# quarterwave0/LithographySimulator

Hardware: AMD Instinct MI355X
Metric: Abbe source-points x image-pixels per second (higher is better)
Workload: dtype f32

## Files before the change

### lithographysimulator_amd/csrc/engine_kernels.hpp

```cpp
#pragma once
#include <hip/hip_runtime.h>

#include "engine_common.hpp"
#include "abbe_plan.hpp"
#include "fft_core.hpp"
#include "wave_fft.hpp"

namespace litho {

template <int LOG2N>
struct Launch {
    using F = LineFFT<LOG2N, +1>;
    static constexpr int L = (F::T >= 64) ? 1 : 64 / F::T;
    static constexpr int THREADS = F::T * L;
#ifndef LITHO_NBUF
#define LITHO_NBUF 1
#endif
    static constexpr int NBUF = (LOG2N <= 12) ? LITHO_NBUF : 1;
    static constexpr size_t LDS_EXCH = (size_t)L * NBUF * F::LDS_LINE;
    static constexpr size_t LDS_BYTES = sizeof(float2) * (LDS_EXCH + F::LDS_TW);
#ifndef LITHO_WG_PER_CU
#define LITHO_WG_PER_CU 3
#endif
    static constexpr int WG_PER_CU = LOG2N <= 12 ? LITHO_WG_PER_CU : (LOG2N == 13 ? 2 : 1);
    static constexpr int WAVES = (THREADS / 256 > 0 ? THREADS / 256 : 1) * WG_PER_CU;
};


typedef unsigned int u32x2 __attribute__((ext_vector_type(2)));
static constexpr unsigned BUF_OOB = 0xFFFF0000u;

__device__ __forceinline__ __amdgpu_buffer_rsrc_t make_rsrc(const void* base, size_t bytes) {
    return __builtin_amdgcn_make_buffer_rsrc(const_cast<void*>(base), 0, (int)(unsigned)bytes, 0x00020000);
}
__device__ __forceinline__ float2 buf_load_c64(__amdgpu_buffer_rsrc_t r, unsigned off) {
    const u32x2 v = __builtin_amdgcn_raw_buffer_load_b64(r, off, 0, 0);
    return make_float2(__uint_as_float(v.x), __uint_as_float(v.y));
}
#ifndef LITHO_XSTORE_AUX
#define LITHO_XSTORE_AUX 16
#endif
template <int LOG2N> inline constexpr int t_store_aux = LOG2N >= 11 ? LITHO_XSTORE_AUX : 0;
typedef unsigned int u32x4 __attribute__((ext_vector_type(4)));
template <int AUX = 0>
__device__ __forceinline__ void buf_store_c64x2(__amdgpu_buffer_rsrc_t r, unsigned off, float2 a, float2 b) {
    u32x4 w;
    w.x = __float_as_uint(a.x); w.y = __float_as_uint(a.y);
    w.z = __float_as_uint(b.x); w.w = __float_as_uint(b.y);
    __builtin_amdgcn_raw_buffer_store_b128(w, r, off, 0, AUX);
}
template <int AUX = 0>
__device__ __forceinline__ void buf_store_c64(__amdgpu_buffer_rsrc_t r, unsigned off, float2 v) {
    u32x2 w;
    w.x = __float_as_uint(v.x);
    w.y = __float_as_uint(v.y);
    __builtin_amdgcn_raw_buffer_store_b64(w, r, off, 0, AUX);
}

__device__ __forceinline__ unsigned t_offset(const PassGeom& g, unsigned a, unsigned q) {
    return ((((q >> g.tcl) * g.rows + a) << g.tcl) + (q & ((1u << g.tcl) - 1u)));
}

typedef unsigned int uint2v __attribute__((ext_vector_type(2)));

__device__ __forceinline__ void touch_vgpr(float2& v) { asm volatile("" : "+v"(v.x), "+v"(v.y)); }
__device__ __forceinline__ void diag_keep(float2 v, unsigned o) { asm volatile("" ::"v"(v.x), "v"(v.y), "v"(o)); }

__device__ __forceinline__ const float* pack_weights() { return nullptr; }
__device__ __forceinline__ const float* pack_weights(const float* w) { return w; }

template <int LOG2N, int RL, bool PRUNED, int NP, int RP = 1, typename... Wt>
__global__ __launch_bounds__(Launch<LOG2N>::THREADS, (RP == 2 ? Launch<LOG2N>::WAVES / Launch<LOG2N>::WG_PER_CU * 2 : Launch<LOG2N>::WAVES)) void k_xpass_abbe(
    const float2* __restrict__ P, const float2* __restrict__ M, const int* __restrict__ shifts,
    float2* __restrict__ Tbuf, const float2* __restrict__ twtab, PassGeom g, int nb, int chunk, Wt... wts)
{
    constexpr bool WT = sizeof...(Wt) != 0;
    static_assert(sizeof...(Wt) <= 1 && !(WT && RP == 2), "weighted x-pass: one weight list, one row per workgroup (a weighted call ignores the row-pair knob)");
    [[maybe_unused]] const float* weights = pack_weights(wts...);
    using F = LineFFT<LOG2N, +1>;
    using LC = Launch<LOG2N>;
    constexpr unsigned IN = PRUNED ? natural_in_mask(RL) : 0xFFFFu;
    constexpr unsigned OUT = out_mask(RL);
    extern __shared__ __attribute__((aligned(16))) unsigned char smem_raw[];
    float2* smem = reinterpret_cast<float2*>(smem_raw);
    const int lt = threadIdx.x % F::T, lg = threadIdx.x / F::T;
    float2* lds = smem + (size_t)lg * LC::NBUF * F::LDS_LINE;

    typename F::Twiddles tw;
    F::load_twiddles(tw, twtab, lt, smem + LC::LDS_EXCH, threadIdx.x, LC::THREADS);

    static_assert(RP == 1 || (RP == 2 && NP == 1 && LC::L == 1), "row pairs: one plane, one line per workgroup");
    int a;
    if constexpr (LC::L == 1) {
        const int b = blockIdx.x, xcd = b & 7, i = b >> 3;
        a = ((i >> 2) * 32 + xcd * 4 + (i & 3)) * RP;
    } else {
        a = blockIdx.x * LC::L + lg;
    }
    const bool active = a < g.rows;
    const bool active1 = a + 1 < g.rows;
    const int r = g.ky0 + g.c + a;
    const size_t plane_bytes = (size_t)g.pn * g.pn * sizeof(float2);
    const __amdgpu_buffer_rsrc_t rM = make_rsrc(M, plane_bytes);

    unsigned koff[16];
    float2 pv[NP * RP][16];
    static_for<0, 16>([&](auto e_) {
        constexpr int e = decltype(e_)::value;
        if constexpr ((IN >> e) & 1u) {
            int k;
            const bool ok = centred_index(lt + F::T * e, F::N, g.kx0, g.kx1, k) && active;
            koff[e] = ok ? (unsigned)(g.c + k) : BUF_OOB;
        }
    });
    static_for<0, NP * RP>([&](auto p_) {
        constexpr int p = decltype(p_)::value;
        const __amdgpu_buffer_rsrc_t rP = make_rsrc(P + (size_t)(RP == 1 ? p : 0) * g.pn * g.pn, plane_bytes);
        static_for<0, 16>([&](auto e_) {
            constexpr int e = decltype(e_)::value;
            if constexpr ((IN >> e) & 1u)
                pv[p][e] = buf_load_c64(rP, koff[e] != BUF_OOB ? ((unsigned)(r + (RP == 1 ? 0 : p)) * g.pn + koff[e]) * 8u : BUF_OOB);
        });
    });
    unsigned toff[16];
    static_for<0, 16>([&](auto m_) {
        constexpr int m = decltype(m_)::value;
        if constexpr ((OUT >> m) & 1u) {
            int u;
            const bool ok = centred_index(lt + F::T * m, F::N, -g.c, g.pn - g.c, u) && active;
            const unsigned q = (unsigned)(u + g.c);
            toff[m] = ok ? t_offset(g, a, q) * 8u : BUF_OOB;
        }
    });

    const int s_begin = blockIdx.y * chunk;
    const int s_end = min(nb, s_begin + chunk);
    auto load_window = [&](int s, int rr, float2 (&mv)[16]) {
        const int dy = shifts[2 * s], dx = shifts[2 * s + 1];
        const unsigned mrow = (unsigned)(r + rr + dy) * g.pn + dx;
        static_for<0, 16>([&](auto e_) {
            constexpr int e = decltype(e_)::value;
            if constexpr ((IN >> e) & 1u)
#ifdef LITHO_DIAG_XNOLOAD
                mv[e] = make_float2((float)((mrow + koff[e]) & 1023u), 1.0f);
#else
                mv[e] = buf_load_c64(rM, koff[e] != BUF_OOB ? (mrow + koff[e]) * 8u : BUF_OOB);
#endif
        });
    };

    int flip = 0;
    float2 mnext[16];
    [[maybe_unused]] float wnext = 1.f;
    if (s_begin < s_end) load_window(s_begin, 0, mnext);
    if constexpr (WT) { if (s_begin < s_end) wnext = weights[s_begin]; }
    static_for<0, 16>([&](auto e_) {
        constexpr int e = decltype(e_)::value;
        if constexpr ((IN >> e) & 1u) touch_vgpr(mnext[e]);
    });
    const unsigned row1 = active1 ? (8u << g.tcl) : 0x80000000u;
    float2 held[RP == 2 ? 16 : 1];
    const bool hi8 = (threadIdx.x & 8) != 0;
    unsigned offc = 0, offd = 0;
    if constexpr (RP == 2) {
        const unsigned tileb = (unsigned)g.rows * (8u << g.tcl);
        offc = hi8 ? row1 - tileb : 0u;
        offd = hi8 ? 0u : row1 + tileb;
    }
    for (int s = s_begin; s < s_end; ++s) {
        static_for<0, RP>([&](auto rr_) {
            constexpr int rr = decltype(rr_)::value;
            float2 mv[16];
            static_for<0, 16>([&](auto e_) {
                constexpr int e = decltype(e_)::value;
                if constexpr ((IN >> e) & 1u) mv[e] = mnext[e];
            });
            [[maybe_unused]] float amp = 1.f;
            if constexpr (WT) amp = sqrtf(wnext);
#ifndef LITHO_XPASS_NO_PREFETCH
            if constexpr (rr + 1 < RP) load_window(s, rr + 1, mnext);
            else load_window(s + 1 < s_end ? s + 1 : s, 0, mnext);
#else
            if constexpr (rr + 1 < RP) load_window(s, rr + 1, mnext);
            else if (s + 1 < s_end) load_window(s + 1, 0, mnext);
#endif
            if constexpr (WT) {
                wnext = weights[s + 1 < s_end ? s + 1 : s];
                static_for<0, 16>([&](auto e_) {
                    constexpr int e = decltype(e_)::value;
                    if constexpr ((IN >> e) & 1u) mv[e] = make_float2(amp * mv[e].x, amp * mv[e].y);
                });
            }
            static_for<0, NP>([&](auto p_) {
                constexpr int p = decltype(p_)::value;
                float2 x[16];
                static_for<0, 16>([&](auto e_) {
                    constexpr int e = decltype(e_)::value;
                    if constexpr ((IN >> e) & 1u) x[e] = cmul(pv[RP == 1 ? p : rr][e], mv[e]);
                    else x[e] = make_float2(0.f, 0.f);
                });
                F::template run<LC::NBUF>(x, tw, lds, lt, flip);
                const __amdgpu_buffer_rsrc_t rT =
                    make_rsrc(Tbuf + ((size_t)p * nb + s) * g.t_point, (size_t)g.t_point * sizeof(float2));
                if constexpr (RP == 2 && rr == 0) {
                    static_for<0, 16>([&](auto m_) { held[decltype(m_)::value] = x[decltype(m_)::value]; });
                } else {
                    static_for<0, 16>([&](auto m_) {
                        constexpr int m = decltype(m_)::value;
#ifdef LITHO_DIAG_XNOSTORE
                        if constexpr ((OUT >> m) & 1u) diag_keep(x[m], toff[m]);
#elif defined(LITHO_DIAG_XSTORE_L2)
                        if constexpr ((OUT >> m) & 1u) buf_store_c64(rT, toff[m] == BUF_OOB ? BUF_OOB : (toff[m] & 0xFFFFFu), x[m]);
#else
                        if constexpr ((OUT >> m) & 1u) {
                            if constexpr (RP == 2) {
                                if (active) {
                                    const float bx = __uint_as_float(__builtin_amdgcn_update_dpp(0u, __float_as_uint(x[m].x), 0x128, 0xF, 0xF, false));
                                    const float by = __uint_as_float(__builtin_amdgcn_update_dpp(0u, __float_as_uint(x[m].y), 0x128, 0xF, 0xF, false));
                                    buf_store_c64<t_store_aux<LOG2N>>(rT, toff[m] + offc, hi8 ? make_float2(bx, by) : held[m]);
                                    buf_store_c64<t_store_aux<LOG2N>>(rT, toff[m] + offd, hi8 ? held[m] : make_float2(bx, by));
                                }
                            } else {
                                buf_store_c64<t_store_aux<LOG2N>>(rT, toff[m], x[m]);
                            }
                        }
#endif
                    });
                }
            });
        });
    }
}

template <int LOG2N, typename... Wt>
__global__ __launch_bounds__(Launch<LOG2N - 1>::THREADS, Launch<LOG2N - 1>::WAVES) void k_xpass_split(
    const float2* __restrict__ P, const float2* __restrict__ M, const int* __restrict__ shifts,
    float2* __restrict__ Tbuf, const float2* __restrict__ twtab, PassGeom g, int nb, int chunk, Wt... wts)
{
    constexpr bool WT = sizeof...(Wt) != 0;
    static_assert(sizeof...(Wt) <= 1, "one weight list");
    [[maybe_unused]] const float* weights = pack_weights(wts...);
    using F = LineFFT<LOG2N - 1, +1>;
    using LC = Launch<LOG2N - 1>;
    static_assert(LC::L == 1, "split x-pass: one row per workgroup");
    constexpr unsigned IN = natural_in_mask(0), OUT = out_mask(1);
    extern __shared__ __attribute__((aligned(16))) unsigned char smem_raw[];
    float2* smem = reinterpret_cast<float2*>(smem_raw);
    const int lt = threadIdx.x;
    float2* lds = smem;

    typename F::Twiddles tw;
    F::load_twiddles(tw, twtab, lt, smem + LC::LDS_EXCH, threadIdx.x, LC::THREADS, 2);

    const int b = blockIdx.x, xcd = b & 7, i = b >> 3;
    const int a = (i >> 2) * 32 + xcd * 4 + (i & 3);
    const bool active = a < g.rows;
    const int r = g.ky0 + g.c + a;
    const size_t plane_bytes = (size_t)g.pn * g.pn * sizeof(float2);
    const __amdgpu_buffer_rsrc_t rM = make_rsrc(M, plane_bytes);
    const __amdgpu_buffer_rsrc_t rP = make_rsrc(P, plane_bytes);

    unsigned koff[16];
    float2 pv0[16], pv1[16];
    static_for<0, 16>([&](auto e_) {
        constexpr int e = decltype(e_)::value;
        if constexpr ((IN >> e) & 1u) {
            int k;
            const bool ok = centred_index(lt + F::T * e, F::N, g.kx0, g.kx1, k) && active;
            koff[e] = ok ? (unsigned)(g.c + k) : BUF_OOB;
            pv0[e] = buf_load_c64(rP, ok ? ((unsigned)r * g.pn + koff[e]) * 8u : BUF_OOB);
            pv1[e] = cmul(pv0[e], twtab[(k + 2 * F::N) & (2 * F::N - 1)]);
        }
    });
    unsigned toff[16];
    static_for<0, 16>([&](auto m_) {
        constexpr int m = decltype(m_)::value;
        if constexpr ((OUT >> m) & 1u) {
            int v;
            const bool ok = centred_index(lt + F::T * m, F::N, -(g.c >> 1), g.c >> 1, v) && active;
            toff[m] = ok ? t_offset(g, a, (unsigned)(2 * v + g.c)) * 8u : BUF_OOB;
        }
    });

    const int s_begin = blockIdx.y * chunk;
    const int s_end = min(nb, s_begin + chunk);
    int flip = 0;
    for (int s = s_begin; s < s_end; ++s) {
        const int dy = shifts[2 * s], dx = shifts[2 * s + 1];
        const unsigned mrow = (unsigned)(r + dy) * g.pn + dx;
        float2 mv[16];
        static_for<0, 16>([&](auto e_) {
            constexpr int e = decltype(e_)::value;
            if constexpr ((IN >> e) & 1u) mv[e] = buf_load_c64(rM, koff[e] != BUF_OOB ? (mrow + koff[e]) * 8u : BUF_OOB);
        });
        if constexpr (WT) {
            const float amp = sqrtf(weights[s]);
            static_for<0, 16>([&](auto e_) {
                constexpr int e = decltype(e_)::value;
                if constexpr ((IN >> e) & 1u) mv[e] = make_float2(amp * mv[e].x, amp * mv[e].y);
            });
        }
        float2 x[16], even[16];
        static_for<0, 16>([&](auto e_) {
            constexpr int e = decltype(e_)::value;
            if constexpr ((IN >> e) & 1u) x[e] = cmul(pv0[e], mv[e]);
            else x[e] = make_float2(0.f, 0.f);
        });
        F::template run<LC::NBUF>(x, tw, lds, lt, flip);
        static_for<0, 16>([&](auto m_) {
            constexpr int m = decltype(m_)::value;
            if constexpr ((OUT >> m) & 1u) even[m] = x[m];
        });
        static_for<0, 16>([&](auto e_) {
            constexpr int e = decltype(e_)::value;
            if constexpr ((IN >> e) & 1u) x[e] = cmul(pv1[e], mv[e]);
            else x[e] = make_float2(0.f, 0.f);
        });
        F::template run<LC::NBUF>(x, tw, lds, lt, flip);
        const __amdgpu_buffer_rsrc_t rT =
            make_rsrc(Tbuf + (size_t)s * g.t_point, (size_t)g.t_point * sizeof(float2));
        static_for<0, 16>([&](auto m_) {
            constexpr int m = decltype(m_)::value;
            if constexpr ((OUT >> m) & 1u) buf_store_c64x2<t_store_aux<LOG2N>>(rT, toff[m], even[m], x[m]);
        });
    }
}

template <int LOG2N, int SIGN, typename Loader>
__global__ __launch_bounds__(Launch<LOG2N>::THREADS, Launch<LOG2N>::WAVES) void k_xpass(
    Loader ld, float2* __restrict__ Tbuf, const float2* __restrict__ twtab, PassGeom g)
{
    using F = LineFFT<LOG2N, SIGN>;
    using LC = Launch<LOG2N>;
    extern __shared__ __attribute__((aligned(16))) unsigned char smem_raw[];
    float2* smem = reinterpret_cast<float2*>(smem_raw);
    const int lt = threadIdx.x % F::T, lg = threadIdx.x / F::T;
    float2* lds = smem + (size_t)lg * LC::NBUF * F::LDS_LINE;

    typename F::Twiddles tw;
// ... 613 lines not shown
```

### lithographysimulator_amd/csrc/wave_fft.hpp

```cpp
#pragma once
#include <hip/hip_runtime.h>

#include "fft_core.hpp"

namespace litho {

static constexpr double W64C[33] = {
    1, 0.99518472667219693, 0.98078528040323043, 0.95694033573220882,
    0.92387953251128674, 0.88192126434835505, 0.83146961230254524, 0.77301045336273699,
    0.70710678118654757, 0.63439328416364549, 0.55557023301960229, 0.47139673682599781,
    0.38268343236508984, 0.29028467725446233, 0.19509032201612833, 0.09801714032956077,
    0.0, -0.098017140329560645, -0.19509032201612819, -0.29028467725446216,
    -0.38268343236508973, -0.4713967368259977, -0.55557023301960196, -0.63439328416364538,
    -0.70710678118654746, -0.77301045336273699, -0.83146961230254535, -0.88192126434835494,
    -0.92387953251128674, -0.95694033573220882, -0.98078528040323043, -0.99518472667219682,
    -1};

template <int M>
__device__ __forceinline__ float2 mul_root64(float2 v)
{
    if constexpr (M == 0) {
        return v;
    } else if constexpr (M == 16) {
        return make_float2(-v.y, v.x);
// ... 118 lines not shown
    struct LaneTwiddles {
        float2 row[NTW];
    };
    __device__ static __forceinline__ void load_lane_twiddles(LaneTwiddles& t, const float2* __restrict__ table, int l, int step)
    {
        static_for<0, 8>([&](auto i_) { constexpr int i = decltype(i_)::value; t.row[i] = table[step * l * i]; });
        static_for<0, S / 8>([&](auto i_) { constexpr int i = decltype(i_)::value; t.row[8 + i] = table[step * l * 8 * i]; });
    }

    static constexpr int TW_LDS_FLOAT2 = NTW * 64;
    __device__ static __forceinline__ void fill_lane_twiddle_table(float2* tab, const float2* __restrict__ table,
                                                                   int step, int tid, int nthreads)
    {
        for (int i = tid; i < TW_LDS_FLOAT2; i += nthreads) {
            const int e = i >> 6, l = i & (S - 1);
            tab[i] = table[e < 8 ? step * l * e : step * l * 8 * (e - 8)];
        }
    }
    template <bool TABLE_FIRST = false>
    __device__ static __forceinline__ void run_lds_tw(float2 (&x)[S], const float2* tab, float* lds, int lane)
    {
        if constexpr (TABLE_FIRST) {
            LaneTwiddles tw;
            asm volatile("" ::: "memory");
            static_for<1, NTW>([&](auto i_) { constexpr int i = decltype(i_)::value; if constexpr (i != 8) tw.row[i] = tab[i * 64 + lane]; });
            run(x, tw, lds, lane);
            return;
        }
        dft_dif(x);
        LaneTwiddles tw;
        asm volatile("" ::: "memory");
        static_for<1, NTW>([&](auto i_) { constexpr int i = decltype(i_)::value; if constexpr (i != 8) tw.row[i] = tab[i * 64 + lane]; });
        run_tail(x, tw, lds, lane);
    }

    __device__ static __forceinline__ void run(float2 (&x)[S], const LaneTwiddles& tw, float* lds, int lane)
    {
        dft_dif(x);
        run_tail(x, tw, lds, lane);
    }
    __device__ static __forceinline__ void lane_twiddle_mul(float2 (&x)[S], const LaneTwiddles& tw)
    {
        static_for<0, S>([&](auto m_) {
            constexpr int m = decltype(m_)::value;
            constexpr int a = m >> 3, b = m & 7, sl = brev(m);
            if constexpr (b != 0) x[sl] = cmul(x[sl], tw.row[b]);
            if constexpr (a != 0) x[sl] = cmul(x[sl], tw.row[8 + a]);
        });
    }
    __device__ static __forceinline__ void run_tail(float2 (&x)[S], const LaneTwiddles& tw, float* lds, int lane)
    {
        lane_twiddle_mul(x, tw);
        transpose(x, lds, lane);
        dft_dif(x);
    }
    __device__ static __forceinline__ void transpose(float2 (&x)[S], float* lds, int lane)
    {
#ifdef LITHO_TRANSPOSE_OPAQUE
        asm volatile("" : "+v"(lane));
#endif
        const int l = lane & (S - 1), line = lane >> LS;
        float* const mat = lds + line * (S * TS);
        float* const wr = mat + l * TS;
        float* const rd = mat + l;
        write_row(wr, [&](auto m_) { return x[brev(decltype(m_)::value)].x; });
        __builtin_amdgcn_fence(__ATOMIC_RELEASE, "wavefront");
        __builtin_amdgcn_wave_barrier();
        float re[S];
        static_for<0, S>([&](auto r_) { constexpr int r = decltype(r_)::value; re[r] = rd[r * TS]; });
        __builtin_amdgcn_fence(__ATOMIC_ACQUIRE, "wavefront");
        __builtin_amdgcn_wave_barrier();
        write_row(wr, [&](auto m_) { return x[brev(decltype(m_)::value)].y; });
        __builtin_amdgcn_fence(__ATOMIC_RELEASE, "wavefront");
        __builtin_amdgcn_wave_barrier();
        static_for<0, S>([&](auto r_) {
            constexpr int r = decltype(r_)::value;
            x[r] = make_float2(re[r], rd[r * TS]);
        });
        __builtin_amdgcn_fence(__ATOMIC_ACQUIRE, "wavefront");
        __builtin_amdgcn_wave_barrier();
    }

    template <int NL>
    __device__ static __forceinline__ void run_rect(float2 (&x)[S], const LaneTwiddles& tw, float* lds, int lane)
    {
        static_assert(LS == 6 && (NL == 2 || NL == 4 || NL == 8 || NL == 16), "rectangular multi-line transform: S = 64");
        constexpr int H = S / NL, LH = LS - (NL == 2 ? 1 : NL == 4 ? 2 : NL == 8 ? 3 : 4);
        static_for<0, NL>([&](auto q_) { dif_network<LH, decltype(q_)::value * H, S>(x); });
        auto slot_of = [](int c) constexpr { return (c / H) * H + brev_bits(c % H, LH); };
        static_for<0, S>([&](auto c_) {
            constexpr int c = decltype(c_)::value;
            constexpr int m = c % H, a = m >> 3, b = m & 7, sl = (c / H) * H + brev_bits(m, LH);
            if constexpr (b != 0) x[sl] = cmul(x[sl], tw.row[b]);
            if constexpr (a != 0) x[sl] = cmul(x[sl], tw.row[8 + a]);
        });
#ifdef LITHO_TRANSPOSE_OPAQUE
        asm volatile("" : "+v"(lane));
#endif
        float* const wr = lds + lane * TS;
        float* const rd = lds + lane;
        write_row(wr, [&](auto c_) { return x[slot_of(decltype(c_)::value)].x; });
        __builtin_amdgcn_fence(__ATOMIC_RELEASE, "wavefront");
        __builtin_amdgcn_wave_barrier();
        float re[S];
        static_for<0, S>([&](auto r_) { constexpr int r = decltype(r_)::value; re[r] = rd[r * TS]; });
        __builtin_amdgcn_fence(__ATOMIC_ACQUIRE, "wavefront");
        __builtin_amdgcn_wave_barrier();
        write_row(wr, [&](auto c_) { return x[slot_of(decltype(c_)::value)].y; });
        __builtin_amdgcn_fence(__ATOMIC_RELEASE, "wavefront");
        __builtin_amdgcn_wave_barrier();
        static_for<0, S>([&](auto r_) {
            constexpr int r = decltype(r_)::value;
            x[r] = make_float2(re[r], rd[r * TS]);
        });
        __builtin_amdgcn_fence(__ATOMIC_ACQUIRE, "wavefront");
        __builtin_amdgcn_wave_barrier();
        dft_dif(x);
    }

    __device__ static __forceinline__ void run_pair(float2 (&x)[S], const LaneTwiddles& tw, float* mat_own,
                                                    const float* mat_other, int lane, int par)
    {
        static_assert(LS == 6, "pair transform: S = 64");
        dft_dif(x);
        static_for<0, S>([&](auto m_) {
            constexpr int m = decltype(m_)::value;
            constexpr int a = m >> 3, b = m & 7, sl = brev(m);
            if constexpr (b != 0) x[sl] = cmul(x[sl], tw.row[b]);
            if constexpr (a != 0) x[sl] = cmul(x[sl], tw.row[8 + a]);
        });
        float* const wr = mat_own + lane * TS;
        const float* const rd0 = (par ? mat_other : mat_own) + lane;
        const float* const rd1 = (par ? mat_own : mat_other) + lane;
        const float sgn = par ? -1.f : 1.f;
        write_row(wr, [&](auto m_) { return x[brev(decltype(m_)::value)].x; });
        lds_barrier();
        float re[S];
        static_for<0, S>([&](auto r_) {
            constexpr int r = decltype(r_)::value;
            re[r] = fmaf(sgn, rd1[r * TS], rd0[r * TS]);
        });
        lds_barrier();
        write_row(wr, [&](auto m_) { return x[brev(decltype(m_)::value)].y; });
        lds_barrier();
        static_for<0, S>([&](auto r_) {
            constexpr int r = decltype(r_)::value;
            x[r] = make_float2(re[r], fmaf(sgn, rd1[r * TS], rd0[r * TS]));
        });
        lds_barrier();
        if (par) static_for<1, S>([&](auto r_) { constexpr int r = decltype(r_)::value; x[r] = mul_root128<r>(x[r]); });
        dft_dif(x);
    }
};

using Wave4096 = WaveSq<6>;

}
```

### lithographysimulator_amd/csrc/wave_kernels.hpp

```cpp
#pragma once
#include "engine_kernels.hpp"

namespace litho {

template <int LOG2N>
struct WaveShape {
    static_assert(LOG2N >= 10 && LOG2N <= 12, "wave-per-line y-pass: N = 1024 .. 4096 (N = 8192: k_ypass_pair)");
    static constexpr int LS = LOG2N / 2;
    static constexpr int D = 1 << (LOG2N - 2 * LS);
    using W = WaveSq<LS>;
    static constexpr int S = W::S;
    static constexpr int THREADS = 256;
    static constexpr int UNITS = THREADS / S;
    static constexpr int COLS = UNITS / D;
    static constexpr int TILES = COLS / 4;
    static constexpr int JLIVE = S * D / 8;
    static constexpr size_t LDS_BYTES = (size_t)(THREADS / 64) * W::LDS_FLOATS * sizeof(float);
#ifndef LITHO_WAVE32_MINWAVES
#define LITHO_WAVE32_MINWAVES 4
#endif
    static constexpr int MINWAVES = LS == 5 ? LITHO_WAVE32_MINWAVES : 2;
};

template <int TC, int COLS>
// ... 394 lines not shown
        if (snext < nb) {
            asm volatile("s_waitcnt lgkmcnt(0)" ::: "memory");
            prefetch(snext);
        }
        W::dft_dif(x);
#endif
        static_for<0, S>([&](auto i_) {
            constexpr int i = decltype(i_)::value;
            const float2 v = x[W::brev(i)];
            acc[i] = fmaf(v.x, v.x, fmaf(v.y, v.y, acc[i]));
        });
    }
    if (!active || qx >= g.pn) return;
    float* srow = slab + ((size_t)grp * g.nt * 4 + qx) * g.pn;
    static_for<0, S>([&](auto i_) {
        constexpr int i = decltype(i_)::value;
        const int n = lane + S * i;
        const int v = n < S * S / 2 ? n : n - S * S;
        srow[v + g.c] += acc[i];
    });
}

template <int LOG2N, int TC>
__global__ __launch_bounds__(256, 2) void k_ypass_pair(
    const float2* __restrict__ Tbuf, float* __restrict__ slab, const float2* __restrict__ twtab,
    PassGeom g, int nb, int G, int gstride)
{
    static_assert(LOG2N == 13, "pair-of-waves y-pass: N = 8192");
    using W = WaveSq<6>;
    constexpr int S = 64, N = 1 << LOG2N;
    extern __shared__ __attribute__((aligned(16))) unsigned char smem_raw[];
    float* smem = reinterpret_cast<float*>(smem_raw);
    const int lane = threadIdx.x & 63;
    const int wv = __builtin_amdgcn_readfirstlane(threadIdx.x >> 6);
    const int par = wv & 1, pair = wv >> 1;
    float* mat_own = smem + wv * W::LDS_FLOATS;
    const float* mat_other = smem + (wv ^ 1) * W::LDS_FLOATS;
    typename W::LaneTwiddles tw;
    W::load_lane_twiddles(tw, twtab, lane + S * par, 1);

    static_assert(TC == 4 || TC == 8, "T tiles are 4 or 8 columns wide");
    const int qx = wave_first_column<TC, 2>(blockIdx.x) + pair;
    const int tile = qx / TC, col = qx & (TC - 1);
    const int plane = blockIdx.y / G, grp = blockIdx.y - plane * G;
    Tbuf += (size_t)plane * nb * g.t_point;
    slab += (size_t)plane * gstride * g.nt * 4 * g.pn;
    const bool active = tile * TC < g.pn;
    float acc[S / 2];
    static_for<0, S / 2>([&](auto i) { acc[i] = 0.f; });

    constexpr int RB = 8 * TC;
    const unsigned tile_bytes = active ? (unsigned)g.rows * RB : 0u;
    const unsigned vb = (unsigned)(lane + S * par - g.ky0) * RB + (unsigned)col * 8u;
    auto slot_off = [&](int j) { return vb + (unsigned)(j <= 8 ? RB * 2 * S * j : RB * 2 * S * j - RB * N); };

    for (int s = grp; s < nb; s += G) {
        const __amdgpu_buffer_rsrc_t rT =
            make_rsrc(Tbuf + (size_t)s * g.t_point + (size_t)(active ? tile : 0) * g.rows * TC, tile_bytes);
        float2 x[S];
        static_for<0, S>([&](auto j_) {
            constexpr int j = decltype(j_)::value;
            if constexpr (j <= 8 || j >= S - 8) x[j] = buf_load_c64(rT, slot_off(j));
            else x[j] = make_float2(0.f, 0.f);
        });
        W::run_pair(x, tw, mat_own, mat_other, lane, par);
        static_for<0, S / 2>([&](auto i_) {
            constexpr int i = decltype(i_)::value;
            constexpr int k2 = i < S / 4 ? i : S / 2 + i;
            const float2 v = x[W::brev(k2)];
            acc[i] = fmaf(v.x, v.x, fmaf(v.y, v.y, acc[i]));
        });
    }

    if (!active || qx >= g.pn) return;
    float* srow = slab + ((size_t)grp * g.nt * 4 + qx) * g.pn;
    static_for<0, S / 2>([&](auto i_) {
        constexpr int i = decltype(i_)::value;
        constexpr int k2 = i < S / 4 ? i : S / 2 + i;
        constexpr int ubase = k2 < S / 2 ? 2 * S * k2 : 2 * S * k2 - N;
        srow[ubase + lane + S * par + g.c] += acc[i];
    });
}

template <int LOG2N, int TC, bool FULL = false, int GW = 1>
__global__ __launch_bounds__(256 * GW, 2) void k_ypass_rect(
    const float2* __restrict__ Tbuf, float* __restrict__ slab, const float2* __restrict__ twtab,
    PassGeom g, int nb, int G, int gstride)
{
    static_assert(GW == 1 || GW == 2, "one or two groups per workgroup");
    static_assert(LOG2N >= 8 && LOG2N <= 11, "multi-column-per-wave y-pass: N = 256 (full output only), 512, 1024, 2048");
    static_assert(TC == 2 || TC == 4 || TC == 8, "T tiles are 2, 4 or 8 columns wide");
    static_assert(LOG2N >= 9 || FULL, "N = 256: the coarse-grid transform of 256^2 images");
    using W = WaveSq<6>;
    constexpr int S = 64, N = 1 << LOG2N, NL = (S * S) / N, H = S / NL;
    constexpr int JL = FULL ? H / 4 : H / 8;
    constexpr int NACC = FULL ? S : S / 2;
    auto kept_k2 = [](int i) constexpr { return FULL ? i : (i < S / 4 ? i : S / 2 + i); };
    static_assert(NL <= TC || NL == 2 * TC, "the wave's columns sit in one T tile, or in two adjacent ones (N = 256)");
    constexpr int NT = NL <= TC ? 1 : 2;
    constexpr int QT = NL / 2 / NT;
    extern __shared__ __attribute__((aligned(16))) unsigned char smem_raw[];
    float* smem = reinterpret_cast<float*>(smem_raw);
    const int lane = threadIdx.x & 63;
    const int wv = __builtin_amdgcn_readfirstlane(threadIdx.x >> 6);
    const int cw = wv & 3, gl = wv >> 2;
    float* lds = smem + wv * W::LDS_FLOATS;
    typename W::LaneTwiddles tw;
    W::load_lane_twiddles(tw, twtab, lane, 1);

    const int qx0 = wave_first_column<TC, 4 * NL>(blockIdx.x) + NL * cw;
    const int tile = qx0 / TC, col = qx0 & (TC - 1);
    const int GB = G / GW;
    const int plane = blockIdx.y / GB, gb = blockIdx.y - plane * GB;
    const int grp = gb * GW + gl;
    Tbuf += (size_t)plane * nb * g.t_point;
    slab += (size_t)plane * gstride * g.nt * 4 * g.pn;
    const bool active = tile * TC < g.pn;
    float acc[NACC];
    static_for<0, NACC>([&](auto i) { acc[i] = 0.f; });

    constexpr int RB = 8 * TC;
    const unsigned tile_bytes = active ? (unsigned)g.rows * RB : 0u;
    const unsigned vb = (unsigned)(lane - g.ky0) * RB + (unsigned)col * 8u;
    auto slot_off = [&](int j) { return vb + (unsigned)(j <= JL ? RB * S * j : RB * S * j - RB * N); };

    for (int s = grp; s < nb; s += G) {
        __amdgpu_buffer_rsrc_t rTs[NT];
        static_for<0, NT>([&](auto t_) {
            constexpr int t = decltype(t_)::value;
            rTs[t] = make_rsrc(Tbuf + (size_t)s * g.t_point + (size_t)(active ? tile + t : 0) * g.rows * TC, tile_bytes);
        });
        float2 x[S];
        static_for<0, H>([&](auto j_) {
            constexpr int j = decltype(j_)::value;
            static_for<0, NL / 2>([&](auto q_) {
                constexpr int q = decltype(q_)::value;
                if constexpr (j <= JL || j >= H - JL) {
                    const u32x4v v = __builtin_amdgcn_raw_buffer_load_b128(rTs[q / QT], slot_off(j) + 16u * (q % QT), 0, LITHO_YLOAD_AUX);
                    x[(2 * q) * H + j] = make_float2(__uint_as_float(v.x), __uint_as_float(v.y));
                    x[(2 * q + 1) * H + j] = make_float2(__uint_as_float(v.z), __uint_as_float(v.w));
                } else {
                    x[(2 * q) * H + j] = make_float2(0.f, 0.f);
                    x[(2 * q + 1) * H + j] = make_float2(0.f, 0.f);
                }
            });
        });
        W::template run_rect<NL>(x, tw, lds, lane);
        static_for<0, NACC>([&](auto i_) {
            constexpr int i = decltype(i_)::value;
            constexpr int k2 = kept_k2(i);
            const float2 v = x[W::brev(k2)];
            acc[i] = fmaf(v.x, v.x, fmaf(v.y, v.y, acc[i]));
        });
    }

    if constexpr (GW == 2) {
        if (gl == 1) static_for<0, NACC>([&](auto i_) { constexpr int i = decltype(i_)::value; lds[i * 64 + lane] = acc[i]; });
        __syncthreads();
        if (gl == 1) return;
        const float* other = smem + (wv + 4) * W::LDS_FLOATS;
        static_for<0, NACC>([&](auto i_) { constexpr int i = decltype(i_)::value; acc[i] += other[i * 64 + lane]; });
    }
    const int qx = qx0 + lane / H, m = lane & (H - 1);
    if (!active || qx >= g.pn) return;
    float* srow = slab + ((size_t)gb * g.nt * 4 + qx) * g.pn;
    static_for<0, NACC>([&](auto i_) {
        constexpr int i = decltype(i_)::value;
        constexpr int k2 = kept_k2(i);
        constexpr int ubase = k2 < S / 2 ? H * k2 : H * k2 - N;
#if defined(LITHO_DIAG_YFLUSH_STORE)
        srow[ubase + m + g.c] = acc[i];
#elif defined(LITHO_DIAG_YFLUSH_NONE)
        if (acc[i] == 12345.678f) srow[ubase + m + g.c] = acc[i];
#else
        srow[ubase + m + g.c] += acc[i];
#endif
    });
}


template <int LOG2N, bool FULL = false, typename... Wt>
__global__ __launch_bounds__(256, 2) void k_xpass_rect(
    const float2* __restrict__ P, const float2* __restrict__ M, const int* __restrict__ shifts,
    float2* __restrict__ Tbuf, const float2* __restrict__ twtab, PassGeom g, int nb, int chunk, Wt... wts)
{
    constexpr bool WT = sizeof...(Wt) != 0;
    static_assert(sizeof...(Wt) <= 1, "one weight list");
    [[maybe_unused]] const float* weights = pack_weights(wts...);
    static_assert(LOG2N >= 9 && LOG2N <= 11, "multi-row-per-wave x-pass: N = 512, 1024, 2048");
    using W = WaveSq<6>;
    constexpr int S = 64, N = 1 << LOG2N, NL = (S * S) / N, H = S / NL, JL = FULL ? H / 4 : H / 8, TC = 8;
    constexpr int NOUT = FULL ? S : S / 2;
    extern __shared__ __attribute__((aligned(16))) unsigned char smem_raw[];
    float* smem = reinterpret_cast<float*>(smem_raw);
    const int lane = threadIdx.x & 63;
    const int wv = __builtin_amdgcn_readfirstlane(threadIdx.x >> 6);
    float* lds = smem + wv * W::LDS_FLOATS;
    typename W::LaneTwiddles tw;
    W::load_lane_twiddles(tw, twtab, lane, 1);

    const int a0 = (blockIdx.x * 4 + wv) * NL;
    const int s_begin = blockIdx.y * chunk;
    const int s_end = min(nb, s_begin + chunk);
    if (a0 >= g.rows) return;

    const unsigned win_bytes = (unsigned)(g.kx1 - g.kx0) * 8u;
    const unsigned vb = (unsigned)(lane - g.kx0) * 8u;
    auto slot_off = [&](int j) { return vb + (unsigned)(j <= JL ? 512 * j : 512 * j - 8 * N); };
    const int r0 = g.ky0 + g.c + a0;

    const int oline = lane / H, om = lane & (H - 1);
    const bool ovalid = a0 + oline < g.rows;
    const unsigned rowstride = (unsigned)g.rows * (TC * 8u);
    const unsigned obase = ovalid ? (unsigned)(om >> 3) * rowstride + (unsigned)(a0 + oline) * (TC * 8u) + (unsigned)(om & 7) * 8u
                                  : BUF_OOB;

    for (int s = s_begin; s < s_end; ++s) {
        const int dy = shifts[2 * s], dx = shifts[2 * s + 1];
        [[maybe_unused]] float amp = 1.f;
        if constexpr (WT) amp = sqrtf(weights[s]);
        float2 x[S];
        static_for<0, NL>([&](auto q_) {
            constexpr int line = decltype(q_)::value;
            const bool rvalid = a0 + line < g.rows;
            const __amdgpu_buffer_rsrc_t rP =
                make_rsrc(P + (size_t)(r0 + (rvalid ? line : 0)) * g.pn + g.c + g.kx0, rvalid ? win_bytes : 0u);
            const __amdgpu_buffer_rsrc_t rM =
                make_rsrc(M + (size_t)(r0 + (rvalid ? line : 0) + dy) * g.pn + dx + g.c + g.kx0, rvalid ? win_bytes : 0u);
            static_for<0, H>([&](auto j_) {
                constexpr int j = decltype(j_)::value;
                if constexpr (j <= JL || j >= H - JL) {
                    if constexpr (WT) {
                        const float2 m = buf_load_c64(rM, slot_off(j));
                        x[line * H + j] = cmul(buf_load_c64(rP, slot_off(j)), make_float2(amp * m.x, amp * m.y));
                    } else {
                        x[line * H + j] = cmul(buf_load_c64(rP, slot_off(j)), buf_load_c64(rM, slot_off(j)));
// ... 6 lines not shown
        const __amdgpu_buffer_rsrc_t rT =
            make_rsrc(Tbuf + (size_t)s * g.t_point, (size_t)g.t_point * sizeof(float2));
        static_for<0, NOUT>([&](auto i_) {
            constexpr int i = decltype(i_)::value;
            constexpr int k2 = FULL ? i : (i < S / 4 ? i : S / 2 + i);
            constexpr int ub = k2 < S / 2 ? H * k2 : H * k2 - N;
            const unsigned tile_off = (unsigned)((ub + g.c) >> 3) * rowstride;
            buf_store_c64(rT, obase == BUF_OOB ? BUF_OOB : obase + tile_off, x[W::brev(k2)]);
        });
    }
}

template <int LOG2N>
hipError_t launch_xpass_rect(const float2* P, const float2* M, const int* shifts, const float* wts, float2* T, const float2* tw,
                             const PassGeom& g, int nb, int chunk, hipStream_t st)
{
    if constexpr (LOG2N >= 9 && LOG2N <= 11) {
        if (g.tcl != 3) return hipErrorNotSupported;
        static LdsOnce once;
        constexpr size_t lds = 4 * WaveSq<6>::LDS_FLOATS * sizeof(float);
        constexpr int NL = 4096 >> LOG2N;
        const int groups = (g.rows + NL - 1) / NL;
        const dim3 grid((groups + 3) / 4, (nb + chunk - 1) / chunk);
        if (wts) {
            if (g.N == g.pn) {
                static LdsOnce once_full_wt;
                auto kern = k_xpass_rect<LOG2N, true, const float*>;
                hipError_t e = set_lds(once_full_wt, kern, lds);
                if (e != hipSuccess) return e;
                hipLaunchKernelGGL(kern, grid, dim3(256), lds, st, P, M, shifts, T, tw, g, nb, chunk, wts);
                note_kernel(0, "k_xpass_rect<%d, true, float const*>", LOG2N);
                return hipGetLastError();
            }
            static LdsOnce once_wt;
            auto kern = k_xpass_rect<LOG2N, false, const float*>;
            hipError_t e = set_lds(once_wt, kern, lds);
            if (e != hipSuccess) return e;
            hipLaunchKernelGGL(kern, grid, dim3(256), lds, st, P, M, shifts, T, tw, g, nb, chunk, wts);
            note_kernel(0, "k_xpass_rect<%d, false, float const*>", LOG2N);
            return hipGetLastError();
        }
        if (g.N == g.pn) {
            static LdsOnce once_full;
            auto kern = k_xpass_rect<LOG2N, true>;
            hipError_t e = set_lds(once_full, kern, lds);
            if (e != hipSuccess) return e;
            hipLaunchKernelGGL(kern, grid, dim3(256), lds, st, P, M, shifts, T, tw, g, nb, chunk);
            note_kernel(0, "k_xpass_rect<%d, true>", LOG2N);
            return hipGetLastError();
        }
        auto kern = k_xpass_rect<LOG2N>;
        hipError_t e = set_lds(once, kern, lds);
        if (e != hipSuccess) return e;
        hipLaunchKernelGGL(kern, grid, dim3(256), lds, st, P, M, shifts, T, tw, g, nb, chunk);
        note_kernel(0, "k_xpass_rect<%d, false>", LOG2N);
        return hipGetLastError();
    } else {
        return hipErrorNotSupported;
    }
}

template <int LOG2N, int TC>
static hipError_t launch_ypass_wave_tc(const float2* T, float* slab, const float2* tw, const PassGeom& g, int nb, int planes, int G,
                     int gstride, hipStream_t st)
{
    constexpr size_t lds4 = 4 * WaveSq<6>::LDS_FLOATS * sizeof(float);
    if (g.N == g.pn) {
        if constexpr (LOG2N == 12) {
            static LdsOnce once;
            constexpr size_t ldsf = lds4 + (size_t)WaveSq<6>::TW_LDS_FLOAT2 * sizeof(float2);
            auto kern = k_ypass_wave<LOG2N, TC, true>;
            hipError_t e = set_lds(once, kern, ldsf);
            if (e != hipSuccess) return e;
            hipLaunchKernelGGL(kern, dim3(wave_grid_x<TC, 4>(g.pn), planes * G), dim3(256), ldsf, st, T, slab, tw, g, nb, G,
                               gstride);
            note_kernel(1, "k_ypass_wave<%d, %d, true>", LOG2N, TC);
            return hipGetLastError();
        } else if constexpr (LOG2N >= 8 && LOG2N <= 11) {
            constexpr int NL = 4096 >> LOG2N;
            if constexpr (NL <= TC || NL == 2 * TC) {
                if (g.gcombine && G % 2 == 0) {
                    static LdsOnce once2;
                    auto kern2 = k_ypass_rect<LOG2N, TC, true, 2>;
                    hipError_t e2 = set_lds(once2, kern2, 2 * lds4);
                    if (e2 != hipSuccess) return e2;
                    hipLaunchKernelGGL(kern2, dim3(wave_grid_x<TC, 4 * NL>(g.pn), planes * (G / 2)), dim3(512), 2 * lds4, st,
                                       T, slab, tw, g, nb, G, gstride);
                    note_kernel(1, "k_ypass_rect<%d, %d, true, 2>", LOG2N, TC);
                    return hipGetLastError();
                }
                static LdsOnce once;
                auto kern = k_ypass_rect<LOG2N, TC, true>;
                hipError_t e = set_lds(once, kern, lds4);
                if (e != hipSuccess) return e;
                hipLaunchKernelGGL(kern, dim3(wave_grid_x<TC, 4 * NL>(g.pn), planes * G), dim3(256), lds4, st, T, slab, tw,
                                   g, nb, G, gstride);
                note_kernel(1, "k_ypass_rect<%d, %d, true, 1>", LOG2N, TC);
                return hipGetLastError();
            }
        }
        return hipErrorNotSupported;
    }
    if constexpr (LOG2N == 13) {
        static LdsOnce once;
        auto kern = k_ypass_pair<LOG2N, TC>;
        hipError_t e = set_lds(once, kern, lds4);
        if (e != hipSuccess) return e;
        hipLaunchKernelGGL(kern, dim3(wave_grid_x<TC, 2>(g.pn), planes * G), dim3(256), lds4, st, T, slab, tw, g, nb, G,
                           gstride);
        note_kernel(1, "k_ypass_pair<%d, %d>", LOG2N, TC);
            return hipGetLastError();
    } else if constexpr (LOG2N >= 9 && LOG2N <= 11) {
        constexpr int NL = 4096 >> LOG2N;
        if constexpr (NL <= TC) {
            if (!g.rect_off) {
                if (g.gcombine && G % 2 == 0) {
                    static LdsOnce once2;
                    auto kern2 = k_ypass_rect<LOG2N, TC, false, 2>;
                    hipError_t e2 = set_lds(once2, kern2, 2 * lds4);
                    if (e2 != hipSuccess) return e2;
                    hipLaunchKernelGGL(kern2, dim3(wave_grid_x<TC, 4 * NL>(g.pn), planes * (G / 2)), dim3(512), 2 * lds4, st,
                                       T, slab, tw, g, nb, G, gstride);
                    note_kernel(1, "k_ypass_rect<%d, %d, false, 2>", LOG2N, TC);
                    return hipGetLastError();
                }
                static LdsOnce once;
                auto kern = k_ypass_rect<LOG2N, TC>;
                hipError_t e = set_lds(once, kern, lds4);
                if (e != hipSuccess) return e;
                hipLaunchKernelGGL(kern, dim3(wave_grid_x<TC, 4 * NL>(g.pn), planes * G), dim3(256), lds4, st, T, slab, tw,
                                   g, nb, G, gstride);
                note_kernel(1, "k_ypass_rect<%d, %d, false, 1>", LOG2N, TC);
                return hipGetLastError();
            }
        }
        if constexpr (LOG2N >= 10) {
            static LdsOnce once;
            using WS = WaveShape<LOG2N>;
            auto kern = k_ypass_wave<LOG2N, TC>;
            hipError_t e = set_lds(once, kern, WS::LDS_BYTES);
            if (e != hipSuccess) return e;
            hipLaunchKernelGGL(kern, dim3(wave_grid_x<TC, WS::COLS>(g.pn), planes * G), dim3(WS::THREADS),
                               WS::LDS_BYTES, st, T, slab, tw, g, nb, G, gstride);
            note_kernel(1, "k_ypass_wave<%d, %d, false>", LOG2N, TC);
            return hipGetLastError();
        } else {
            return hipErrorNotSupported;
        }
    } else if constexpr (LOG2N == 12) {
        static LdsOnce once;
        using WS = WaveShape<LOG2N>;
        auto kern = k_ypass_wave<LOG2N, TC>;
        hipError_t e = set_lds(once, kern, WS::LDS_BYTES);
        if (e != hipSuccess) return e;
        hipLaunchKernelGGL(kern, dim3(wave_grid_x<TC, WS::COLS>(g.pn), planes * G), dim3(WS::THREADS), WS::LDS_BYTES,
                           st, T, slab, tw, g, nb, G, gstride);
        note_kernel(1, "k_ypass_wave<%d, %d, false>", LOG2N, TC);
        return hipGetLastError();
    } else {
        return hipErrorNotSupported;
    }
}

template <int LOG2N>
hipError_t launch_ypass_wave(const float2* T, float* slab, const float2* tw, const PassGeom& g, int nb, int planes,
                             int G, int gstride, hipStream_t st)
{
    if (g.tcl == 2) return launch_ypass_wave_tc<LOG2N, 4>(T, slab, tw, g, nb, planes, G, gstride, st);
    if (g.tcl == 3) return launch_ypass_wave_tc<LOG2N, 8>(T, slab, tw, g, nb, planes, G, gstride, st);
    if constexpr (LOG2N == 12) {
        if (g.tcl == 4 && g.N == g.pn) {
#ifndef LITHO_COOP_WAVES
#define LITHO_COOP_WAVES 4
#endif
            constexpr int NW = LITHO_COOP_WAVES;
            if (g.coop_dma) {
#ifndef LITHO_COOP_DMA_WAVES
#define LITHO_COOP_DMA_WAVES 4
#endif
                constexpr int ND = LITHO_COOP_DMA_WAVES;
                static LdsOnce once_dma;
                auto kd = k_ypass_coop_dma<LOG2N, ND>;
                hipError_t ed = set_lds(once_dma, kd, CoopDmaShape<ND>::LDS_BYTES);
                if (ed != hipSuccess) return ed;
                hipLaunchKernelGGL(kd, dim3(CoopDmaShape<ND>::grid_x(g.pn), planes * G), dim3(64 * ND), CoopDmaShape<ND>::LDS_BYTES, st, T,
                                   slab, tw, g, nb, G, gstride);
                note_kernel(1, "k_ypass_coop_dma<%d, %d>", LOG2N, ND);
                return hipGetLastError();
            }
            static LdsOnce once;
            auto kern = k_ypass_coop<LOG2N, NW>;
            hipError_t e = set_lds(once, kern, CoopShape<NW>::LDS_BYTES);
            if (e != hipSuccess) return e;
            hipLaunchKernelGGL(kern, dim3(CoopShape<NW>::grid_x(g.pn), planes * G), dim3(64 * NW), CoopShape<NW>::LDS_BYTES, st, T,
                               slab, tw, g, nb, G, gstride);
            note_kernel(1, "k_ypass_coop<%d, %d>", LOG2N, NW);
            return hipGetLastError();
        }
    }
    return hipErrorNotSupported;
}

#define LITHO_DEFINE_WAVE_OPS(L2)                                                                            \
    template hipError_t launch_ypass_wave<L2>(const float2*, float*, const float2*, const PassGeom&, int, int, int, \
                                              int, hipStream_t);                                             \
    template hipError_t launch_xpass_rect<L2>(const float2*, const float2*, const int*, const float*, float2*, const float2*,  \
                                              const PassGeom&, int, int, hipStream_t);

}
```

Measured before the change: 504.7 billion.

## Read rect y-pass twiddles from an LDS table; exit idle x-pass workgroups early

For the rectangular y-pass at small NL (H>=16), per-lane factored twiddles held in registers are replaced by a full twiddle table built in LDS once per workgroup and read per element. The fill happens after the first item's loads are issued so it overlaps them. This cuts register pressure and one of the two complex multiplies per element, at the cost of extra LDS space and LDS reads. Separately, x-pass workgroups with no active rows now return before loading twiddles, so padding blocks no longer do useless work.

Measured after the change: 498.9 billion. -1.1%, worse.

```diff
diff --git a/lithographysimulator_amd/csrc/engine_kernels.hpp b/lithographysimulator_amd/csrc/engine_kernels.hpp
--- a/lithographysimulator_amd/csrc/engine_kernels.hpp
+++ b/lithographysimulator_amd/csrc/engine_kernels.hpp
@@ -86,9 +86,6 @@
     const int lt = threadIdx.x % F::T, lg = threadIdx.x / F::T;
     float2* lds = smem + (size_t)lg * LC::NBUF * F::LDS_LINE;
 
-    typename F::Twiddles tw;
-    F::load_twiddles(tw, twtab, lt, smem + LC::LDS_EXCH, threadIdx.x, LC::THREADS);
-
     static_assert(RP == 1 || (RP == 2 && NP == 1 && LC::L == 1), "row pairs: one plane, one line per workgroup");
     int a;
     if constexpr (LC::L == 1) {
@@ -99,6 +96,11 @@
     }
     const bool active = a < g.rows;
     const bool active1 = a + 1 < g.rows;
+#ifndef LITHO_XPASS_PAD_RUNS
+    if (LC::L == 1 ? !active : (int)blockIdx.x * LC::L >= g.rows) return;
+#endif
+    typename F::Twiddles tw;
+    F::load_twiddles(tw, twtab, lt, smem + LC::LDS_EXCH, threadIdx.x, LC::THREADS);
     const int r = g.ky0 + g.c + a;
     const size_t plane_bytes = (size_t)g.pn * g.pn * sizeof(float2);
     const __amdgpu_buffer_rsrc_t rM = make_rsrc(M, plane_bytes);
@@ -249,12 +251,14 @@
     const int lt = threadIdx.x;
     float2* lds = smem;
 
-    typename F::Twiddles tw;
-    F::load_twiddles(tw, twtab, lt, smem + LC::LDS_EXCH, threadIdx.x, LC::THREADS, 2);
-
     const int b = blockIdx.x, xcd = b & 7, i = b >> 3;
     const int a = (i >> 2) * 32 + xcd * 4 + (i & 3);
     const bool active = a < g.rows;
+#ifndef LITHO_XPASS_PAD_RUNS
+    if (!active) return;
+#endif
+    typename F::Twiddles tw;
+    F::load_twiddles(tw, twtab, lt, smem + LC::LDS_EXCH, threadIdx.x, LC::THREADS, 2);
     const int r = g.ky0 + g.c + a;
     const size_t plane_bytes = (size_t)g.pn * g.pn * sizeof(float2);
     const __amdgpu_buffer_rsrc_t rM = make_rsrc(M, plane_bytes);
diff --git a/lithographysimulator_amd/csrc/wave_fft.hpp b/lithographysimulator_amd/csrc/wave_fft.hpp
--- a/lithographysimulator_amd/csrc/wave_fft.hpp
+++ b/lithographysimulator_amd/csrc/wave_fft.hpp
@@ -224,18 +224,17 @@
     }
 
     template <int NL>
-    __device__ static __forceinline__ void run_rect(float2 (&x)[S], const LaneTwiddles& tw, float* lds, int lane)
+    __device__ static __forceinline__ void rect_pass_a(float2 (&x)[S])
     {
         static_assert(LS == 6 && (NL == 2 || NL == 4 || NL == 8 || NL == 16), "rectangular multi-line transform: S = 64");
         constexpr int H = S / NL, LH = LS - (NL == 2 ? 1 : NL == 4 ? 2 : NL == 8 ? 3 : 4);
         static_for<0, NL>([&](auto q_) { dif_network<LH, decltype(q_)::value * H, S>(x); });
+    }
+    template <int NL>
+    __device__ static __forceinline__ void rect_tail(float2 (&x)[S], float* lds, int lane)
+    {
+        constexpr int H = S / NL, LH = LS - (NL == 2 ? 1 : NL == 4 ? 2 : NL == 8 ? 3 : 4);
         auto slot_of = [](int c) constexpr { return (c / H) * H + brev_bits(c % H, LH); };
-        static_for<0, S>([&](auto c_) {
-            constexpr int c = decltype(c_)::value;
-            constexpr int m = c % H, a = m >> 3, b = m & 7, sl = (c / H) * H + brev_bits(m, LH);
-            if constexpr (b != 0) x[sl] = cmul(x[sl], tw.row[b]);
-            if constexpr (a != 0) x[sl] = cmul(x[sl], tw.row[8 + a]);
-        });
 #ifdef LITHO_TRANSPOSE_OPAQUE
         asm volatile("" : "+v"(lane));
 #endif
@@ -258,6 +257,47 @@
         __builtin_amdgcn_fence(__ATOMIC_ACQUIRE, "wavefront");
         __builtin_amdgcn_wave_barrier();
         dft_dif(x);
+    }
+    template <int NL>
+    __device__ static __forceinline__ void run_rect(float2 (&x)[S], const LaneTwiddles& tw, float* lds, int lane)
+    {
+        constexpr int H = S / NL, LH = LS - (NL == 2 ? 1 : NL == 4 ? 2 : NL == 8 ? 3 : 4);
+        rect_pass_a<NL>(x);
+        static_for<0, S>([&](auto c_) {
+            constexpr int c = decltype(c_)::value;
+            constexpr int m = c % H, a = m >> 3, b = m & 7, sl = (c / H) * H + brev_bits(m, LH);
+            if constexpr (b != 0) x[sl] = cmul(x[sl], tw.row[b]);
+            if constexpr (a != 0) x[sl] = cmul(x[sl], tw.row[8 + a]);
+        });
+        rect_tail<NL>(x, lds, lane);
+    }
+
+    template <int NL>
+    static constexpr int RECT_TW_FLOAT2 = (S / NL - 1) * 64;
+    template <int NL, int NTHREADS>
+    __device__ static __forceinline__ void fill_rect_twiddle_table(float2* tab, const float2* __restrict__ table, int tid)
+    {
+        constexpr int CNT = RECT_TW_FLOAT2<NL>;
+        static_for<0, (CNT + NTHREADS - 1) / NTHREADS>([&](auto k_) {
+            const int i = tid + decltype(k_)::value * NTHREADS;
+            if (i < CNT) tab[i] = table[(i & 63) * ((i >> 6) + 1)];
+        });
+    }
+    template <int NL>
+    __device__ static __forceinline__ void run_rect_tab(float2 (&x)[S], const float2* tab, float* lds, int lane)
+    {
+        constexpr int H = S / NL, LH = LS - (NL == 2 ? 1 : NL == 4 ? 2 : NL == 8 ? 3 : 4);
+        rect_pass_a<NL>(x);
+        asm volatile("" ::: "memory");
+        static_for<1, H>([&](auto m_) {
+            constexpr int m = decltype(m_)::value;
+            const float2 w = tab[(m - 1) * 64 + lane];
+            static_for<0, NL>([&](auto q_) {
+                constexpr int sl = decltype(q_)::value * H + brev_bits(m, LH);
+                x[sl] = cmul(x[sl], w);
+            });
+        });
+        rect_tail<NL>(x, lds, lane);
     }
 
     __device__ static __forceinline__ void run_pair(float2 (&x)[S], const LaneTwiddles& tw, float* mat_own,
diff --git a/lithographysimulator_amd/csrc/wave_kernels.hpp b/lithographysimulator_amd/csrc/wave_kernels.hpp
--- a/lithographysimulator_amd/csrc/wave_kernels.hpp
+++ b/lithographysimulator_amd/csrc/wave_kernels.hpp
@@ -500,6 +500,21 @@
     });
 }
 
+template <int LOG2N, int GW>
+struct RectLds {
+    static constexpr int NL = 4096 >> LOG2N, H = 64 / NL;
+    static constexpr size_t MAT_BYTES = (size_t)4 * GW * WaveSq<6>::LDS_FLOATS * sizeof(float);
+    static constexpr size_t CU_LDS = 160 * 1024;
+    static constexpr size_t TAB_BYTES = (size_t)WaveSq<6>::template RECT_TW_FLOAT2<NL> * sizeof(float2);
+#ifdef LITHO_LANE_TW_FACTORED
+    static constexpr bool TABLE = false;
+#else
+    static constexpr bool TABLE = H >= 16 && (2 / GW) * (MAT_BYTES + TAB_BYTES) <= CU_LDS;
+#endif
+    static constexpr size_t BYTES = MAT_BYTES + (TABLE ? TAB_BYTES : 0);
+    static_assert((2 / GW) * BYTES <= CU_LDS, "8 waves per CU: the workgroups' LDS stays within the 160 KB of a CU");
+};
+
 template <int LOG2N, int TC, bool FULL = false, int GW = 1>
 __global__ __launch_bounds__(256 * GW, 2) void k_ypass_rect(
     const float2* __restrict__ Tbuf, float* __restrict__ slab, const float2* __restrict__ twtab,
@@ -523,8 +538,10 @@
     const int wv = __builtin_amdgcn_readfirstlane(threadIdx.x >> 6);
     const int cw = wv & 3, gl = wv >> 2;
     float* lds = smem + wv * W::LDS_FLOATS;
-    typename W::LaneTwiddles tw;
-    W::load_lane_twiddles(tw, twtab, lane, 1);
+    constexpr bool TABLE = RectLds<LOG2N, GW>::TABLE;
+    [[maybe_unused]] typename W::LaneTwiddles tw;
+    [[maybe_unused]] float2* const twlds = reinterpret_cast<float2*>(smem_raw + RectLds<LOG2N, GW>::MAT_BYTES);
+    if constexpr (!TABLE) W::load_lane_twiddles(tw, twtab, lane, 1);
 
     const int qx0 = wave_first_column<TC, 4 * NL>(blockIdx.x) + NL * cw;
     const int tile = qx0 / TC, col = qx0 & (TC - 1);
@@ -542,6 +559,54 @@
     const unsigned vb = (unsigned)(lane - g.ky0) * RB + (unsigned)col * 8u;
     auto slot_off = [&](int j) { return vb + (unsigned)(j <= JL ? RB * S * j : RB * S * j - RB * N); };
 
+    auto load_item = [&](int s, float2 (&x)[S]) {
+        __amdgpu_buffer_rsrc_t rTs[NT];
+        static_for<0, NT>([&](auto t_) {
+            constexpr int t = decltype(t_)::value;
+            rTs[t] = make_rsrc(Tbuf + (size_t)s * g.t_point + (size_t)(active ? tile + t : 0) * g.rows * TC, tile_bytes);
+        });
+        static_for<0, H>([&](auto j_) {
+            constexpr int j = decltype(j_)::value;
+            static_for<0, NL / 2>([&](auto q_) {
+                constexpr int q = decltype(q_)::value;
+                if constexpr (j <= JL || j >= H - JL) {
+                    const u32x4v v = __builtin_amdgcn_raw_buffer_load_b128(rTs[q / QT], slot_off(j) + 16u * (q % QT), 0, LITHO_YLOAD_AUX);
+                    x[(2 * q) * H + j] = make_float2(__uint_as_float(v.x), __uint_as_float(v.y));
+                    x[(2 * q + 1) * H + j] = make_float2(__uint_as_float(v.z), __uint_as_float(v.w));
+                } else {
+                    x[(2 * q) * H + j] = make_float2(0.f, 0.f);
+                    x[(2 * q + 1) * H + j] = make_float2(0.f, 0.f);
+                }
+            });
+        });
+    };
+    auto accumulate = [&](float2 (&x)[S]) {
+        static_for<0, NACC>([&](auto i_) {
+            constexpr int i = decltype(i_)::value;
+            constexpr int k2 = kept_k2(i);
+            const float2 v = x[W::brev(k2)];
+            acc[i] = fmaf(v.x, v.x, fmaf(v.y, v.y, acc[i]));
+        });
+    };
+
+    if constexpr (TABLE) {
+        bool fill = true;
+        if (grp >= nb) {
+            W::template fill_rect_twiddle_table<NL, 256 * GW>(twlds, twtab, threadIdx.x);
+            __syncthreads();
+        }
+        for (int s = grp; s < nb; s += G) {
+            float2 x[S];
+            load_item(s, x);
+            if (fill) {
+                W::template fill_rect_twiddle_table<NL, 256 * GW>(twlds, twtab, threadIdx.x);
+                __syncthreads();
+                fill = false;
+            }
+            W::template run_rect_tab<NL>(x, twlds, lds, lane);
+            accumulate(x);
+        }
+    } else {
     for (int s = grp; s < nb; s += G) {
         __amdgpu_buffer_rsrc_t rTs[NT];
         static_for<0, NT>([&](auto t_) {
@@ -570,6 +635,7 @@
             const float2 v = x[W::brev(k2)];
             acc[i] = fmaf(v.x, v.x, fmaf(v.y, v.y, acc[i]));
         });
+    }
     }
 
     if constexpr (GW == 2) {
@@ -742,18 +808,20 @@
                 if (g.gcombine && G % 2 == 0) {
                     static LdsOnce once2;
                     auto kern2 = k_ypass_rect<LOG2N, TC, true, 2>;
-                    hipError_t e2 = set_lds(once2, kern2, 2 * lds4);
+                    constexpr size_t ldsr2 = RectLds<LOG2N, 2>::BYTES;
+                    hipError_t e2 = set_lds(once2, kern2, ldsr2);
                     if (e2 != hipSuccess) return e2;
-                    hipLaunchKernelGGL(kern2, dim3(wave_grid_x<TC, 4 * NL>(g.pn), planes * (G / 2)), dim3(512), 2 * lds4, st,
+                    hipLaunchKernelGGL(kern2, dim3(wave_grid_x<TC, 4 * NL>(g.pn), planes * (G / 2)), dim3(512), ldsr2, st,
                                        T, slab, tw, g, nb, G, gstride);
                     note_kernel(1, "k_ypass_rect<%d, %d, true, 2>", LOG2N, TC);
                     return hipGetLastError();
                 }
                 static LdsOnce once;
                 auto kern = k_ypass_rect<LOG2N, TC, true>;
-                hipError_t e = set_lds(once, kern, lds4);
+                constexpr size_t ldsr1 = RectLds<LOG2N, 1>::BYTES;
+                hipError_t e = set_lds(once, kern, ldsr1);
                 if (e != hipSuccess) return e;
-                hipLaunchKernelGGL(kern, dim3(wave_grid_x<TC, 4 * NL>(g.pn), planes * G), dim3(256), lds4, st, T, slab, tw,
+                hipLaunchKernelGGL(kern, dim3(wave_grid_x<TC, 4 * NL>(g.pn), planes * G), dim3(256), ldsr1, st, T, slab, tw,
                                    g, nb, G, gstride);
                 note_kernel(1, "k_ypass_rect<%d, %d, true, 1>", LOG2N, TC);
                 return hipGetLastError();
@@ -777,18 +845,20 @@
                 if (g.gcombine && G % 2 == 0) {
                     static LdsOnce once2;
                     auto kern2 = k_ypass_rect<LOG2N, TC, false, 2>;
-                    hipError_t e2 = set_lds(once2, kern2, 2 * lds4);
+                    constexpr size_t ldsr2 = RectLds<LOG2N, 2>::BYTES;
+                    hipError_t e2 = set_lds(once2, kern2, ldsr2);
                     if (e2 != hipSuccess) return e2;
-                    hipLaunchKernelGGL(kern2, dim3(wave_grid_x<TC, 4 * NL>(g.pn), planes * (G / 2)), dim3(512), 2 * lds4, st,
+                    hipLaunchKernelGGL(kern2, dim3(wave_grid_x<TC, 4 * NL>(g.pn), planes * (G / 2)), dim3(512), ldsr2, st,
                                        T, slab, tw, g, nb, G, gstride);
                     note_kernel(1, "k_ypass_rect<%d, %d, false, 2>", LOG2N, TC);
                     return hipGetLastError();
                 }
                 static LdsOnce once;
                 auto kern = k_ypass_rect<LOG2N, TC>;
-                hipError_t e = set_lds(once, kern, lds4);
+                constexpr size_t ldsr1 = RectLds<LOG2N, 1>::BYTES;
+                hipError_t e = set_lds(once, kern, ldsr1);
                 if (e != hipSuccess) return e;
-                hipLaunchKernelGGL(kern, dim3(wave_grid_x<TC, 4 * NL>(g.pn), planes * G), dim3(256), lds4, st, T, slab, tw,
+                hipLaunchKernelGGL(kern, dim3(wave_grid_x<TC, 4 * NL>(g.pn), planes * G), dim3(256), ldsr1, st, T, slab, tw,
                                    g, nb, G, gstride);
                 note_kernel(1, "k_ypass_rect<%d, %d, false, 1>", LOG2N, TC);
                 return hipGetLastError();
```
